# kartikmadhira1/YA_VO

Hardware: AMD Instinct MI355X
Metric: frames/sec (detect+describe+match+PnP) on 1241×376 KITTI stereo; RMSE vs CPU ref (higher is better)
Workload: dtype u8

## Files before the change

### ya_vo_amd/csrc/yavo_kernels.hip

```cpp
#include <hip/hip_runtime.h>
#include <stdint.h>
#include <stdlib.h>
#include <string.h>

#include "yavo_xlane.h"
#include "yavo_internal.h"


namespace yavo {

__device__ __forceinline__ int lane_id() { return (int)(threadIdx.x & 63); }

__device__ __forceinline__ int wave_incl_scan(int v) {
    v += __builtin_amdgcn_update_dpp(0, v, 0x111, 0xf, 0xf, false);
    v += __builtin_amdgcn_update_dpp(0, v, 0x112, 0xf, 0xf, false);
    v += __builtin_amdgcn_update_dpp(0, v, 0x114, 0xf, 0xf, false);
    v += __builtin_amdgcn_update_dpp(0, v, 0x118, 0xf, 0xf, false);
    v += __builtin_amdgcn_update_dpp(0, v, 0x142, 0xa, 0xf, false);
    v += __builtin_amdgcn_update_dpp(0, v, 0x143, 0xc, 0xf, false);
    return v;
}

template <int NT>
__device__ __forceinline__ int block_excl_scan(int v, int* s_tmp, int* total) {
    const int lane = lane_id();
    const int wave = (int)threadIdx.x >> 6;
    constexpr int NW = NT / 64;
    int incl = wave_incl_scan(v);
    if (lane == 63) s_tmp[wave] = incl;
    __syncthreads();
    if (wave == 0) {
        int w = lane < NW ? s_tmp[lane] : 0;
        int wi = wave_incl_scan(w);
        if (lane < NW) s_tmp[lane] = wi - w;
        if (lane == NW - 1) s_tmp[NW] = wi;
    }
    __syncthreads();
    int res = s_tmp[wave] + incl - v;
    if (total) *total = s_tmp[NW];
    __syncthreads();
    return res;
}

#define YV_RING_DR {0, 1, 2, 3, 3, 3, 2, 1, 0, -1, -2, -3, -3, -3, -2, -1}
#define YV_RING_DC {-3, -3, -2, -1, 0, 1, 2, 3, 3, 3, 2, 1, 0, -1, -2, -3}

__device__ __forceinline__ float cv_hypotf(float a, float b) {
    a = fabsf(a);
    b = fabsf(b);
    if (a > b) {
        b /= a;
        return a * sqrtf(1.0f + b * b);
    }
    if (b > 0.0f) {
        a /= b;
        return b * sqrtf(1.0f + a * a);
    }
    return 0.0f;
}

__device__ __forceinline__ float eig_hypotf(float x, float y) {
    x = fabsf(x);
    y = fabsf(y);
    if (isinf(x) || isinf(y)) return __builtin_inff();
    if (isnan(x) || isnan(y)) return __builtin_nanf("");
    const float p = x > y ? x : y;
    if (p == 0.0f) return 0.0f;
    const float qp = (y < x ? y : x) / p;
    return p * sqrtf(1.0f + qp * qp);
}

__device__ void eig_selfadjoint2(float m00, float m01, float m11, float& w0, float& w1) {
    float scale = fabsf(m00);
    if (fabsf(m01) > scale) scale = fabsf(m01);
    if (fabsf(m11) > scale) scale = fabsf(m11);
    if (scale == 0.0f) scale = 1.0f;
    float d0 = m00 / scale, d1 = m11 / scale, e = m01 / scale;
    int iter = 0, ok = 1;
    while (true) {
        if (fabsf(e) < 1.17549435082228750797e-38f) {
            e = 0.0f;
        } else {
            const float se = 8388608.0f * e;
            if (se * se <= (fabsf(d0) + fabsf(d1))) e = 0.0f;
        }
        if (e == 0.0f) break;
        if (++iter > 60) { ok = 0; break; }
        const float td = (d0 - d1) * 0.5f;
        float mu = d1;
        if (td == 0.0f) {
            mu -= fabsf(e);
        } else {
            const float e2 = e * e;
            const float h = eig_hypotf(td, e);
            if (e2 == 0.0f) mu -= e / ((td + (td > 0.0f ? h : -h)) / e);
            else mu -= e2 / (td + (td > 0.0f ? h : -h));
        }
        const float x = d0 - mu, z = e;
        float c, sn;
        if (x == 0.0f) {
            c = 0.0f;
            sn = z < 0.0f ? 1.0f : -1.0f;
        } else if (fabsf(x) > fabsf(z)) {
            const float t = z / x;
            float u = sqrtf(1.0f + t * t);
            if (x < 0.0f) u = -u;
            c = 1.0f / u;
            sn = -t * c;
        } else {
            const float t = x / z;
            float u = sqrtf(1.0f + t * t);
            if (z < 0.0f) u = -u;
            sn = -1.0f / u;
            c = -t * sn;
        }
        const float sdk = sn * d0 + c * e;
        const float dkp1 = sn * e + c * d1;
        const float nd0 = c * (c * d0 - sn * e) - sn * (c * e - sn * d1);
        const float nd1 = sn * sdk + c * dkp1;
        const float ne = c * sdk - sn * dkp1;
        d0 = nd0;
        d1 = nd1;
        e = ne;
    }
    if (ok && d1 < d0) { const float t = d0; d0 = d1; d1 = t; }
    d0 *= scale;
    d1 *= scale;
    w0 = d1;
    w1 = d0;
}

__device__ __forceinline__ float harris_response(float a, float b, float d, int eig) {
    float w0 = a, w1 = d;
    if (eig == 1) {
        eig_selfadjoint2(a, b, d, w0, w1);
    } else if (!(fabsf(b) <= 1.1920928955078125e-07f)) {
        const float p = b;
        const float y = (float)((double)(w1 - w0) * 0.5);
        float t = fabsf(y) + cv_hypotf(p, y);
        float s = cv_hypotf(p, t);
        s = p / s;
        t = (p / t) * p;
        if (y < 0.0f) { s = -s; t = -t; }
        w0 -= t;
        w1 += t;
    }
    if (eig != 1 && w0 < w1) { float tmp = w0; w0 = w1; w1 = tmp; }
    const float prod = w0 * w1;
    const float sum = w1 + w0;
    const double sq = (double)sum * (double)sum;
    const double r = (double)prod - 0.04 * sq;
    return (float)r;
}

__device__ __forceinline__ uint64_t make_key(float resp, uint32_t idx) {
    if (resp == 0.0f) resp = 0.0f;
    uint32_t u = __float_as_uint(resp);
    uint32_t ord = (u & 0x80000000u) ? ~u : (u | 0x80000000u);
    return ((uint64_t)(~ord) << 32) | (uint64_t)idx;
}
__device__ __forceinline__ float key_resp(uint64_t key) {
    uint32_t ord = ~(uint32_t)(key >> 32);
    uint32_t u = (ord & 0x80000000u) ? (ord & 0x7fffffffu) : ~ord;
    return __uint_as_float(u);
}

struct K9 {
    uint32_t k[9];
    uint32_t kh[4][3];
    uint32_t kve[5];
    uint32_t kvo[5];
    int byte2;
    int mfma;
    int hbias;
};

static K9 make_k9(const uint16_t* k9) {
    K9 kw = {};
    uint32_t sum = 0;
    for (int i = 0; i < 9; ++i) {
        kw.k[i] = k9[i];
        sum += k9[i];
    }
    auto tap = [&](int t) -> uint32_t { return (t >= 0 && t <= 8) ? (uint32_t)k9[t] : 0u; };
    for (int j = 0; j < 4; ++j)
        for (int m = 0; m < 3; ++m)
            for (int i = 0; i < 4; ++i) kw.kh[j][m] |= tap(4 * m + i - j) << (8 * i);
    for (int t = 0; t < 5; ++t) {
        kw.kve[t] = tap(2 * t) | (tap(2 * t + 1) << 16);
        kw.kvo[t] = tap(2 * t - 1) | (tap(2 * t) << 16);
    }
    kw.byte2 = sum <= 256 ? 1 : 0;
    uint32_t mx = 0;
    for (int i = 0; i < 9; ++i) mx = k9[i] > mx ? k9[i] : mx;
    kw.mfma = mx <= 127 ? 1 : 0;
    kw.hbias = (int)(128 * sum);
    return kw;
}

__device__ __forceinline__ int reflect101(int p, int len) {
    if (p < 0) p = -p;
    if (p >= len) p = 2 * len - p - 2;
    return p;
}

#ifdef YAVO_LM_PROFILE
constexpr int kDetProfSlots = 131072;
__device__ unsigned long long g_det_prof[kDetProfSlots][6];
#define DP_DECL unsigned long long dp_acc[6] = {0, 0, 0, 0, 0, 0}; unsigned long long dp_t = __builtin_readcyclecounter();
#define DP_MARK(k) do { const unsigned long long t_ = __builtin_readcyclecounter(); dp_acc[k] += t_ - dp_t; dp_t = t_; } while (0)
#define DP_STORE() do { \
        const unsigned slot_ = blockIdx.x; \
        if (threadIdx.x == 0 && slot_ < kDetProfSlots) for (int q_ = 0; q_ < 6; ++q_) g_det_prof[slot_][q_] = dp_acc[q_]; \
    } while (0)
#else
#define DP_DECL
#define DP_MARK(k) do {} while (0)
#define DP_STORE() do {} while (0)
#endif
#ifdef YAVO_LM_PROFILE
constexpr int kBriefProfSlots = 16384;
__device__ unsigned long long g_brief_prof[kBriefProfSlots][6];
#define BP_DECL unsigned long long bp_acc[4] = {0, 0, 0, 0}; unsigned long long bp_t = __builtin_readcyclecounter(); \
    const unsigned long long bp_rt0 = __builtin_amdgcn_s_memrealtime();
#define BP_MARK(k) do { const unsigned long long t_ = __builtin_readcyclecounter(); bp_acc[k] += t_ - bp_t; bp_t = t_; } while (0)
#define BP_STORE() do { \
        if (threadIdx.x == 0 && blockIdx.x < kBriefProfSlots) { \
            g_brief_prof[blockIdx.x][0] = bp_acc[0] + bp_acc[1]; g_brief_prof[blockIdx.x][1] = bp_acc[2]; \
            g_brief_prof[blockIdx.x][2] = bp_rt0; \
            g_brief_prof[blockIdx.x][3] = __builtin_amdgcn_s_memrealtime(); \
            g_brief_prof[blockIdx.x][4] = (unsigned long long)__builtin_amdgcn_s_getreg(0xF804); \
            g_brief_prof[blockIdx.x][5] = (unsigned long long)__builtin_amdgcn_s_getreg(0xF814); \
        } \
    } while (0)
#else
#define BP_DECL
#define BP_MARK(k) do {} while (0)
#define BP_STORE() do {} while (0)
#endif
constexpr int FT_W = kFastTileW;
constexpr int FT_H = kFastTileH;
constexpr int FT_R = 4;
constexpr int FT_LW = FT_W + 2 * FT_R;
constexpr int FT_LH = FT_H + 2 * FT_R;

template <bool kBlur>
__global__ __launch_bounds__(256) void detect_kernel(const uint8_t* __restrict__ imgs, int H, int W, int stride,
                                                     int64_t pitch, int thr, int eig, uint64_t* __restrict__ cand_keys,
                                                     int64_t cap, uint32_t* __restrict__ cand_count, K9 kw,
                                                     uint8_t* __restrict__ blur) {
    __shared__ __align__(16) uint8_t tile[FT_LH * FT_LW];
    constexpr int kPreDw = FT_W * FT_H / 2, kHbufDw = kBlur ? (FT_LH / 2) * FT_W : 0;
    __shared__ __align__(16) uint32_t s_share[kPreDw > kHbufDw ? kPreDw : kHbufDw];
    uint16_t* s_pre = reinterpret_cast<uint16_t*>(s_share);
    uint32_t* hbuf = s_share;
    __shared__ uint16_t s_pos[FT_W * FT_H];
    __shared__ uint32_t s_n, s_npre, s_base;
    __shared__ uint32_t s_band[4 * 9];
    DP_DECL
    const int ntx = (W + FT_W - 1) / FT_W, nty = (H + FT_H - 1) / FT_H;
    const int lb = xcd_swizzle((int)blockIdx.x, (int)gridDim.x);
    const int img = lb / (ntx * nty), tyx = lb - img * (ntx * nty);
    const int r0 = (tyx / ntx) * FT_H, c0 = (tyx % ntx) * FT_W;
    const uint8_t* src = imgs + (int64_t)img * pitch;
    const int tid = threadIdx.x;
    const int lane = lane_id();
    const int wave = tid >> 6;
    if (tid == 0) {
        s_n = 0;
        s_npre = 0;
    }
    if (kBlur && tid < 4 * 9) {
        const int r = tid / 9, M = tid - 9 * r - 3;
        uint32_t v = 0;
#pragma unroll
        for (int j = 0; j < 4; ++j)
#pragma unroll
            for (int m = 0; m < 3; ++m)
                if (r == j && M == m) v = kw.kh[j][m];
        s_band[tid] = v;
    }

    {
        constexpr int kDw = FT_LW / 4;
        constexpr int kSlots = FT_LH * kDw;
        constexpr int kPer = (kSlots + 255) / 256;
        const bool interior = (c0 >= FT_R) && (c0 + FT_W + FT_R <= W) && (r0 >= FT_R) && (r0 + FT_H + FT_R < H);
        uint32_t v[kPer];
        if (interior) {
            const uint8_t* base = src + (int64_t)(r0 - FT_R) * stride + (c0 - FT_R);
            const int lr0 = tid / kDw, j0 = tid - lr0 * kDw;
            uint32_t off = (uint32_t)(lr0 * stride + 4 * j0);
            int j = j0;
            const uint32_t step = (uint32_t)(14 * stride + 16), wrap = (uint32_t)(15 * stride - 56);
            const uint32_t last = (uint32_t)((kSlots - 1) / kDw * stride + 4 * ((kSlots - 1) % kDw));
#pragma unroll
            for (int u = 0; u < kPer; ++u) {
                const uint32_t o = (256 * u + 255 >= kSlots && tid + 256 * u >= kSlots) ? last : off;
                __builtin_memcpy(&v[u], base + o, 4);
                const bool c = j + 4 >= kDw;
                off += c ? wrap : step;
                j += c ? 4 - kDw : 4;
            }
        } else {
#pragma unroll
            for (int u = 0; u < kPer; ++u) {
                const int t = min(tid + 256 * u, kSlots - 1);
                const int lr = t / kDw, j = t - lr * kDw;
                const int r = reflect101(min(max(r0 - FT_R + lr, -(H - 1)), 2 * H - 2), H);
                const uint8_t* row = src + (int64_t)r * stride;
                const int cc = c0 - FT_R + 4 * j;
                if (cc >= 0 && cc + 4 <= W) {
                    __builtin_memcpy(&v[u], row + cc, 4);
                } else {
                    uint32_t w = 0;
#pragma unroll
                    for (int b = 0; b < 4; ++b)
                        w |= (uint32_t)row[reflect101(min(max(cc + b, -(W - 1)), 2 * W - 2), W)] << (8 * b);
                    v[u] = w;
                }
            }
        }
        uint32_t* tile32 = reinterpret_cast<uint32_t*>(tile);
#pragma unroll
        for (int u = 0; u < kPer; ++u) {
            const int t = tid + 256 * u;
            if (t < kSlots) tile32[t] = v[u];
        }
    }
    __syncthreads();
    DP_MARK(0);

    constexpr int ring_dr[16] = YV_RING_DR;
    constexpr int ring_dc[16] = YV_RING_DC;
    const uint32_t neg_thr = (uint32_t)(-thr);
    const int tx = lane;
    const int ty = __builtin_amdgcn_readfirstlane(wave);
    const int c = c0 + tx;
    constexpr int kRowIters = FT_H / 4;
    uint32_t row_ok = 0;
#pragma unroll
    for (int u = 0; u < kRowIters; ++u) row_ok |= (uint32_t)((unsigned)(r0 + ty + 4 * u - 4) < (unsigned)(H - 8)) << u;
    uint32_t nmask = 0;
    const uint8_t* wbase = &tile[(ty + FT_R - 3) * FT_LW + tx + FT_R - 3];
#pragma unroll
    for (int u = kRowIters - 1; u >= 0; --u) {
        const uint8_t* t0 = wbase + 4 * u * FT_LW;
        const uint32_t cent = t0[3 * FT_LW + 3];
        auto d = [&](int k) {
            return __builtin_amdgcn_sad_u8(cent, (uint32_t)t0[(ring_dr[k] + 3) * FT_LW + ring_dc[k] + 3], neg_thr);
        };
        const uint32_t v = (d(0) | d(4)) | (d(8) | d(11));
        nmask = __builtin_amdgcn_alignbit(nmask, v, 31);
    }
    uint32_t pmask = (unsigned)(c - 4) < (unsigned)(W - 8) ? (~nmask & row_ok) : 0u;
    {
        const int cnt = __popc(pmask);
        const int incl = wave_incl_scan(cnt);
        const int total = __shfl(incl, 63, 64);
        uint32_t base = 0;
        if (lane == 0 && total > 0) base = atomicAdd(&s_npre, (uint32_t)total);
        base = __shfl(base, 0, 64);
        uint32_t off = base + (uint32_t)(incl - cnt);
        while (pmask) {
            const int u = __builtin_ctz(pmask);
            s_pre[off++] = (uint16_t)((ty + 4 * u) * FT_W + tx);
            pmask &= pmask - 1;
        }
    }
    __syncthreads();
    DP_MARK(1);
    const uint32_t npre = s_npre;
    for (uint32_t i0 = 0; i0 < npre; i0 += 256) {
        const uint32_t i = i0 + tid;
        bool cand = false;
        int pos = 0;
        if (i < npre) {
            pos = s_pre[i];
            const uint8_t* t0 = &tile[((pos >> 6) + FT_R - 3) * FT_LW + (pos & 63) + FT_R - 3];
            const uint32_t cent = t0[3 * FT_LW + 3];
            uint32_t sim = 0;
#pragma unroll
            for (int k = 0; k < 16; ++k)
                sim = __builtin_amdgcn_alignbit(
                    sim, __builtin_amdgcn_sad_u8(cent, (uint32_t)t0[(ring_dr[k] + 3) * FT_LW + ring_dc[k] + 3], neg_thr),
                    31);
            const uint32_t mask = ~sim & 0xFFFFu;
            const uint32_t a2 = mask & (mask >> 1);
            const uint32_t a4 = a2 & (a2 >> 2);
            const uint32_t a8 = a4 & (a4 >> 4);
            const uint32_t a12 = a8 & (a4 >> 8);
            cand = a12 != 0u;
        }
        const uint64_t bal = __ballot(cand);
        if (bal == 0) continue;
        const int leader = __ffsll((long long)bal) - 1;
        uint32_t base = 0;
        if (lane == leader) base = atomicAdd(&s_n, (uint32_t)__popcll(bal));
        base = __shfl(base, leader, 64);
        if (cand) s_pos[base + (uint32_t)__popcll(bal & ((1ull << lane) - 1ull))] = (uint16_t)pos;
    }
    __syncthreads();
    DP_MARK(2);
    const uint32_t n = s_n;
    if (tid == 0 && n > 0) s_base = atomicAdd(&cand_count[img], n);
    if (kBlur && kw.mfma) {
        typedef int dt_v4i __attribute__((ext_vector_type(4)));
        const int n = lane & 15, g = lane >> 4;
        dt_v4i B;
#pragma unroll
        for (int jj = 0; jj < 4; ++jj) {
            const int M = 4 * g + jj - (n >> 2);
            B[jj] = (M >= -3 && M <= 5) ? (int)s_band[(n & 3) * 9 + M + 3] : 0;
        }
        const dt_v4i C = {kw.hbias, kw.hbias, kw.hbias, kw.hbias};
        const int rb = ty;
        const uint8_t* arow = &tile[(16 * rb + n) * FT_LW + 16 * g];
#pragma unroll
        for (int cb = 0; cb < 4; ++cb) {
            const uint2 lo = *reinterpret_cast<const uint2*>(arow + 16 * cb);
            const uint2 hi = *reinterpret_cast<const uint2*>(arow + 16 * cb + 8);
            const dt_v4i A = {(int)(lo.x ^ 0x80808080u), (int)(lo.y ^ 0x80808080u), (int)(hi.x ^ 0x80808080u),
                              (int)(hi.y ^ 0x80808080u)};
            const dt_v4i acc = __builtin_amdgcn_mfma_i32_16x16x64_i8(A, B, C, 0, 0, 0);
            const int q = 8 * rb + 2 * g, x = 16 * cb + n;
            hbuf[q * FT_W + x] = (uint32_t)acc[0] | ((uint32_t)acc[1] << 16);
            hbuf[(q + 1) * FT_W + x] = (uint32_t)acc[2] | ((uint32_t)acc[3] << 16);
        }
    } else if (kBlur) {
        const uint32_t* trow = reinterpret_cast<const uint32_t*>(tile);
        constexpr int kItems = (FT_LH / 2) * (FT_W / 4);
        for (int i = tid; i < kItems; i += 256) {
            const int q = i >> 4, xq = (i & 15) * 4;
            uint32_t hv[2][4];
#pragma unroll
            for (int h = 0; h < 2; ++h) {
                const uint32_t* wr = trow + ((2 * q + h) * FT_LW >> 2) + (xq >> 2);
                const uint32_t d0 = wr[0], d1 = wr[1], d2 = wr[2];
#pragma unroll
                for (int j = 0; j < 4; ++j) {
                    uint32_t acc = __builtin_amdgcn_udot4(d0, kw.kh[j][0], 0u, false);
                    acc = __builtin_amdgcn_udot4(d1, kw.kh[j][1], acc, false);
                    hv[h][j] = __builtin_amdgcn_udot4(d2, kw.kh[j][2], acc, false);
                }
            }
            *reinterpret_cast<uint4*>(&hbuf[q * FT_W + xq]) =
                make_uint4(hv[0][0] | (hv[1][0] << 16), hv[0][1] | (hv[1][1] << 16), hv[0][2] | (hv[1][2] << 16),
                           hv[0][3] | (hv[1][3] << 16));
        }
    }
    __syncthreads();
    DP_MARK(3);
    if (n > 0) {
        uint64_t* out = cand_keys + (int64_t)img * cap + s_base;
        for (uint32_t i = tid; i < n; i += 256) {
            const int pos = s_pos[i];
            const int prr = pos >> 6, ptx = pos & 63;
            const uint8_t* t0 = &tile[(prr + FT_R - 2) * FT_LW + ptx + FT_R - 2];
            int sxx = 0, sxy = 0, syy = 0;
#pragma unroll
            for (int ii = -1; ii <= 1; ++ii) {
#pragma unroll
                for (int j = -1; j <= 1; ++j) {
                    const uint8_t* q = t0 + (ii + 2) * FT_LW + j + 2;
                    const int pmm = q[-FT_LW - 1], pm0 = q[-FT_LW], pmp = q[-FT_LW + 1];
                    const int p0m = q[-1], p0p = q[1];
                    const int ppm = q[FT_LW - 1], pp0 = q[FT_LW], ppp = q[FT_LW + 1];
                    const int gx = (pmp - pmm) + 2 * (p0p - p0m) + (ppp - ppm);
                    const int gy = (ppm - pmm) + 2 * (pp0 - pm0) + (ppp - pmp);
                    sxx += gx * gx;
                    sxy += gx * gy;
                    syy += gy * gy;
                }
            }
            const float resp = harris_response((float)sxx, (float)sxy, (float)syy, eig);
            out[i] = make_key(resp, (uint32_t)((r0 + prr) * W + (c0 + ptx)));
        }
    }
    DP_MARK(4);
    if (kBlur) {
        typedef unsigned short us2 __attribute__((ext_vector_type(2)));
        const int bp = blur_pitch(W);
        uint8_t* dst = blur + (int64_t)img * H * bp;
        for (int i = tid; i < (FT_H / 2) * (FT_W / 4); i += 256) {
            const int m = i >> 4, xq = (i & 15) * 4;
            uint4 P[5];
#pragma unroll
            for (int t = 0; t < 5; ++t) {
                typedef unsigned int u32x4 __attribute__((ext_vector_type(4)));
                typedef const volatile __attribute__((address_space(3))) u32x4 lds_u32x4;
                const u32x4 q = *(lds_u32x4*)(&s_share[(m + t) * FT_W + xq]);
                P[t] = make_uint4(q.x, q.y, q.z, q.w);
            }
            uint32_t ev[4], od[4];
#pragma unroll
            for (int j = 0; j < 4; ++j) {
                auto col = [&](const uint4& q) { return j == 0 ? q.x : j == 1 ? q.y : j == 2 ? q.z : q.w; };
                uint32_t e = 1u << 15, o = 1u << 15;
#pragma unroll
                for (int t = 0; t < 5; ++t) {
                    e = __builtin_amdgcn_udot2(__builtin_bit_cast(us2, col(P[t])), __builtin_bit_cast(us2, kw.kve[t]), e, false);
                    o = __builtin_amdgcn_udot2(__builtin_bit_cast(us2, col(P[t])), __builtin_bit_cast(us2, kw.kvo[t]), o, false);
                }
                ev[j] = e;
                od[j] = o;
            }
            uint32_t w0, w1;
            if (kw.byte2) {
                w0 = __builtin_amdgcn_perm(__builtin_amdgcn_perm(ev[3], ev[2], 0x0c0c0602u),
                                           __builtin_amdgcn_perm(ev[1], ev[0], 0x0c0c0602u), 0x05040100u);
                w1 = __builtin_amdgcn_perm(__builtin_amdgcn_perm(od[3], od[2], 0x0c0c0602u),
                                           __builtin_amdgcn_perm(od[1], od[0], 0x0c0c0602u), 0x05040100u);
            } else {
                w0 = w1 = 0;
#pragma unroll
                for (int j = 0; j < 4; ++j) {
                    w0 |= min(ev[j] >> 16, 255u) << (8 * j);
                    w1 |= min(od[j] >> 16, 255u) << (8 * j);
                }
            }
            const int r = r0 + 2 * m, c = c0 + xq;
            if (r < H) *reinterpret_cast<uint32_t*>(&dst[(int64_t)r * bp + c]) = w0;
            if (r + 1 < H) *reinterpret_cast<uint32_t*>(&dst[(int64_t)(r + 1) * bp + c]) = w1;
        }
    }
    DP_MARK(5);
    DP_STORE();
}

void launch_fast_harris(const uint8_t* imgs, int n_images, int H, int W, int stride, int64_t pitch,
                        int thr, int eig, uint64_t* cand_keys, int64_t cap, uint32_t* cand_count, hipStream_t s) {
    dim3 grid(((W + FT_W - 1) / FT_W) * ((H + FT_H - 1) / FT_H) * n_images);
    K9 kw = {};
    hipLaunchKernelGGL(detect_kernel<false>, grid, dim3(256), 0, s, imgs, H, W, stride, pitch, thr, eig, cand_keys,
                       cap, cand_count, kw, (uint8_t*)nullptr);
}

void launch_detect_blur(const uint8_t* imgs, int n_images, int H, int W, int stride, int64_t pitch, int thr,
                        int eig, uint64_t* cand_keys, int64_t cap, uint32_t* cand_count, const uint16_t* k9_host,
                        uint8_t* blur, hipStream_t s) {
    dim3 grid(((W + FT_W - 1) / FT_W) * ((H + FT_H - 1) / FT_H) * n_images);
    const K9 kw = make_k9(k9_host);
    hipLaunchKernelGGL(detect_kernel<true>, grid, dim3(256), 0, s, imgs, H, W, stride, pitch, thr, eig, cand_keys, cap,
                       cand_count, kw, blur);
}

constexpr int BL_W = 64, BL_H = 32, BL_R = 4;
constexpr int BL_LW = BL_W + 2 * BL_R;
constexpr int BL_LH = BL_H + 2 * BL_R;

__global__ __launch_bounds__(256) void blur9_kernel(const uint8_t* __restrict__ imgs, int H, int W, int stride,
                                                    int64_t pitch, K9 kw, uint8_t* __restrict__ blur) {
    __shared__ uint8_t tin[BL_LH * BL_LW];
    __shared__ uint32_t th[BL_LH * BL_W];
    const int img = blockIdx.z;
    const int r0 = blockIdx.y * BL_H, c0 = blockIdx.x * BL_W;
    const uint8_t* src = imgs + (int64_t)img * pitch;
    const int tid = threadIdx.x;
    for (int i = tid; i < BL_LH * BL_LW; i += 256) {
        const int lr = i / BL_LW, lc = i - lr * BL_LW;
        const int r = reflect101(min(max(r0 - BL_R + lr, -(H - 1)), 2 * H - 2), H);
        const int c = reflect101(min(max(c0 - BL_R + lc, -(W - 1)), 2 * W - 2), W);
        tin[i] = src[(int64_t)r * stride + c];
    }
    __syncthreads();
    for (int i = tid; i < BL_LH * BL_W; i += 256) {
        const int lr = i >> 6, lc = i & 63;
        const uint8_t* q = &tin[lr * BL_LW + lc];
        uint32_t acc = 0;
#pragma unroll
        for (int j = 0; j < 9; ++j) acc += kw.k[j] * (uint32_t)q[j];
        th[i] = acc;
    }
    __syncthreads();
    const int tx = tid & 63, ty = tid >> 6;
    const int c = c0 + tx;
    for (int rr = ty; rr < BL_H; rr += 4) {
        const int r = r0 + rr;
        uint32_t acc = 0;
#pragma unroll
        for (int i = 0; i < 9; ++i) acc += kw.k[i] * th[(rr + i) * BL_W + tx];
        uint32_t v = (acc + (1u << 15)) >> 16;
        if (r < H && c < W) blur[(int64_t)img * blur_image_bytes(H, W) + (int64_t)r * blur_pitch(W) + c] = (uint8_t)(v > 255u ? 255u : v);
    }
}

void launch_blur9(const uint8_t* imgs, int n_images, int H, int W, int stride, int64_t pitch,
                  const uint16_t* k9_host, uint8_t* blur, hipStream_t s) {
    const K9 kw = make_k9(k9_host);
    dim3 grid((W + BL_W - 1) / BL_W, (H + BL_H - 1) / BL_H, n_images);
    hipLaunchKernelGGL(blur9_kernel, grid, dim3(256), 0, s, imgs, H, W, stride, pitch, kw, blur);
}

constexpr int TK_NT = 1024;

__device__ __forceinline__ bool brief_boundary(int row, int col, int H, int W) {
    return !(col - 8 < 0 || col + 8 > W) && !(row - 8 < 0 || row + 8 > H);
}

__host__ __device__ constexpr int bank_classes(int nb) { return nb <= kBandCounters / 32 ? 32 : 1; }

template <int NT, class RcAt>
__device__ void boundary_compact(RcAt rc_at, int K, int H, int W, int32_t* kp_src, int32_t* kp_count,
                                 int32_t* kp_band, int32_t* band_off, int* s_tmp, int* s_band) {
    const int tid = threadIdx.x;
    const int nb = (H + kBandRows - 1) / kBandRows;
    const int C = bank_classes(nb), nbc = nb * C;
    const int LS = brief_lds_stride(W);
    auto bucket = [&](int row, int col) -> int {
        const int band = row / kBandRows;
        const int cls = C == 1 ? 0 : ((((row - band * kBandRows + 8) * LS + col) >> 2) & 31);
        return band * C + cls;
    };
    for (int b = tid; b < nbc; b += NT) s_band[b] = 0;
    __syncthreads();
    int base = 0;
    for (int pass = 0; pass < 2; ++pass) {
        base = 0;
        for (int c0 = 0; c0 < K; c0 += 4 * NT) {
            int flags[4];
            int2 rcs[4];
            int cnt = 0;
#pragma unroll
            for (int u = 0; u < 4; ++u) {
                const int i = c0 + tid * 4 + u;
                flags[u] = 0;
                rcs[u] = make_int2(0, 0);
                if (i < K) {
                    rcs[u] = rc_at(i);
                    flags[u] = brief_boundary(rcs[u].x, rcs[u].y, H, W) ? 1 : 0;
                }
                cnt += flags[u];
            }
            int total = 0;
            int off = base + block_excl_scan<NT>(cnt, s_tmp, &total);
#pragma unroll
            for (int u = 0; u < 4; ++u) {
                const int i = c0 + tid * 4 + u;
                if (flags[u]) {
                    const int bk = bucket(rcs[u].x, rcs[u].y);
                    if (pass == 0) {
                        reinterpret_cast<int4*>(kp_src)[off] = make_int4(rcs[u].x, rcs[u].y, i, 0);
                        atomicAdd(&s_band[bk], 1);
                    } else {
                        const int pos = atomicAdd(&s_band[bk], 1);
                        reinterpret_cast<int4*>(kp_band)[pos] = make_int4(rcs[u].x, rcs[u].y, i, off);
                    }
                    off++;
                }
            }
            base += total;
        }
        __syncthreads();
        if (pass == 0) {
            int acc = 0;
            for (int b0 = 0; b0 < nbc; b0 += NT) {
                const int j = b0 + tid;
                const int c = j < nbc ? s_band[j] : 0;
                int tot = 0;
                const int first = acc + block_excl_scan<NT>(c, s_tmp, &tot);
                if (j < nbc) {
                    s_band[j] = first;
                    if (j % C == 0) band_off[j / C] = first;
                }
                acc += tot;
            }
            if (tid == 0) band_off[nb] = acc;
        }
        __syncthreads();
    }
    if (tid == 0) *kp_count = base;
}

constexpr int TK_SEL_NT = 512;
static_assert(TK_SEL_NT >= 256 && TK_SEL_NT % 64 == 0, "the radix-select histogram scan uses the first 256 threads");
template <int NT>
__global__ __launch_bounds__(NT) void topk_kernel(const uint64_t* __restrict__ cand_keys, int64_t cap,
                                                     uint32_t* __restrict__ cand_count, uint32_t* __restrict__ cand_seen,
                                                     int H, int W, int max_kp, int keep, int32_t* __restrict__ det_rc,
                                                     float* __restrict__ det_resp, int32_t* __restrict__ det_count,
                                                     int32_t* __restrict__ kp_src, int32_t* __restrict__ kp_count,
                                                     int32_t* __restrict__ kp_band, int32_t* __restrict__ band_off) {
    __shared__ uint64_t s_keys[kMaxKp];
    __shared__ uint32_t s_hist[256];
    __shared__ int s_tmp[40];
    __shared__ int s_band[kBandCounters];
    __shared__ uint64_t s_prefix, s_mask;
    __shared__ int s_krem, s_done, s_n;

    const int img = blockIdx.x;
    const int tid = threadIdx.x;
    const uint64_t* keys = cand_keys + (int64_t)img * cap;
    int64_t C64 = (int64_t)cand_count[img];
    if (C64 > cap) C64 = cap;
    const int C = (int)C64;
    const int K = C < keep ? C : keep;
    __syncthreads();
    if (tid == 0) {
        cand_seen[img] = (uint32_t)C;
        cand_count[img] = 0;
    }
    int32_t* rc_out = det_rc + (int64_t)img * max_kp * 2;
    float* resp_out = det_resp + (int64_t)img * max_kp;

    if (K == 0) {
        const int nb = (H + kBandRows - 1) / kBandRows;
        for (int b = tid; b <= nb; b += NT) band_off[(int64_t)img * (kMaxBands + 1) + b] = 0;
        if (tid == 0) { det_count[img] = 0; kp_count[img] = 0; }
        return;
    }
    uint64_t sel_mask = 0, sel_prefix = ~0ull;
    if (C > K) {
        if (tid == 0) { s_prefix = 0; s_mask = 0; s_krem = K; s_done = 0; }
        __syncthreads();
        for (int shift = 56; shift >= 0; shift -= 8) {
            const uint64_t pm = s_mask, pp = s_prefix;
            const int krem = s_krem;
            if (tid < 256) s_hist[tid] = 0;
            __syncthreads();
            for (int i = tid; i < C; i += NT) {
                const uint64_t k = keys[i];
                if ((k & pm) == pp) atomicAdd(&s_hist[(k >> shift) & 255u], 1u);
            }
            __syncthreads();
            int h = 0, incl = 0;
            if (tid < 256) {
                h = (int)s_hist[tid];
                incl = wave_incl_scan(h);
                if ((tid & 63) == 63) s_tmp[tid >> 6] = incl;
            }
            __syncthreads();
            if (tid < 256) {
                int base = 0;
                for (int w = 0; w < (tid >> 6); ++w) base += s_tmp[w];
                incl += base;
                if (incl >= krem && incl - h < krem) {
                    const int nk = krem - (incl - h);
                    s_prefix = pp | ((uint64_t)tid << shift);
                    s_mask = pm | (0xFFull << shift);
                    s_krem = nk;
                    s_done = (h == nk);
                }
            }
            __syncthreads();
            if (s_done) break;
        }
        sel_mask = s_mask;
        sel_prefix = s_prefix;
    }
    if (tid == 0) s_n = 0;
    __syncthreads();
    for (int i = tid; i < C; i += NT) {
        const uint64_t k = keys[i];
        if ((k & sel_mask) <= sel_prefix) {
            const int p = atomicAdd(&s_n, 1);
            if (p < kMaxKp) s_keys[p] = k;
        }
    }
    __syncthreads();
    int P2 = 1;
    while (P2 < K) P2 <<= 1;
    for (int i = K + tid; i < P2; i += NT) s_keys[i] = ~0ull;
    __syncthreads();
    for (int size = 2; size <= P2; size <<= 1) {
        for (int stride = size >> 1; stride > 0; stride >>= 1) {
            for (int t = tid; t < (P2 >> 1); t += NT) {
                const int i = 2 * t - (t & (stride - 1));
                const int j = i + stride;
                const bool up = ((i & size) == 0);
                const uint64_t a = s_keys[i], b = s_keys[j];
                if ((a > b) == up) { s_keys[i] = b; s_keys[j] = a; }
            }
            __syncthreads();
        }
    }
    for (int i = tid; i < K; i += NT) {
        const uint64_t k = s_keys[i];
        const uint32_t idx = (uint32_t)k;
        const int row = (int)(idx / (uint32_t)W), col = (int)(idx - (uint32_t)row * (uint32_t)W);
        rc_out[2 * i] = row;
        rc_out[2 * i + 1] = col;
// ... 758 lines not shown
```

Baseline: 245,700.

## Compute separable Gaussian blur entirely with MFMA in detect kernel

When the blur kernel is normalized (sum 256) with small taps, the horizontal pass is done by MFMA into registers and the vertical pass is also done by MFMA, with the intermediate split into low and high byte planes so it fits the int8 path. The result is staged in swizzled shared memory and written straight to the blur output, and the kernel returns early, skipping the separate vertical-blur pass and one LDS round trip of the horizontal buffer. Harris scoring is moved into a lambda so both paths can share it. The MFMA path is now restricted to kernels whose taps sum to 256; other kernels fall back to the udot4 path. The byte-split arithmetic adds risk of rounding mismatches against the CPU reference.

```diff
diff --git a/ya_vo_amd/csrc/yavo_kernels.hip b/ya_vo_amd/csrc/yavo_kernels.hip
--- a/ya_vo_amd/csrc/yavo_kernels.hip
+++ b/ya_vo_amd/csrc/yavo_kernels.hip
@@ -193,7 +193,7 @@
     kw.byte2 = sum <= 256 ? 1 : 0;
     uint32_t mx = 0;
     for (int i = 0; i < 9; ++i) mx = k9[i] > mx ? k9[i] : mx;
-    kw.mfma = mx <= 127 ? 1 : 0;
+    kw.mfma = (mx <= 127 && sum == 256) ? 1 : 0;
     kw.hbias = (int)(128 * sum);
     return kw;
 }
@@ -256,7 +256,8 @@
     uint32_t* hbuf = s_share;
     __shared__ uint16_t s_pos[FT_W * FT_H];
     __shared__ uint32_t s_n, s_npre, s_base;
-    __shared__ uint32_t s_band[4 * 9];
+    constexpr int kBandM = 19;
+    __shared__ uint32_t s_band[4 * kBandM];
     DP_DECL
     const int ntx = (W + FT_W - 1) / FT_W, nty = (H + FT_H - 1) / FT_H;
     const int lb = xcd_swizzle((int)blockIdx.x, (int)gridDim.x);
@@ -270,8 +271,8 @@
         s_n = 0;
         s_npre = 0;
     }
-    if (kBlur && tid < 4 * 9) {
-        const int r = tid / 9, M = tid - 9 * r - 3;
+    if (kBlur && tid < 4 * kBandM) {
+        const int r = tid / kBandM, M = tid - kBandM * r - 3;
         uint32_t v = 0;
 #pragma unroll
         for (int j = 0; j < 4; ++j)
@@ -403,56 +404,8 @@
     __syncthreads();
     DP_MARK(2);
     const uint32_t n = s_n;
-    if (tid == 0 && n > 0) s_base = atomicAdd(&cand_count[img], n);
-    if (kBlur && kw.mfma) {
-        typedef int dt_v4i __attribute__((ext_vector_type(4)));
-        const int n = lane & 15, g = lane >> 4;
-        dt_v4i B;
-#pragma unroll
-        for (int jj = 0; jj < 4; ++jj) {
-            const int M = 4 * g + jj - (n >> 2);
-            B[jj] = (M >= -3 && M <= 5) ? (int)s_band[(n & 3) * 9 + M + 3] : 0;
-        }
-        const dt_v4i C = {kw.hbias, kw.hbias, kw.hbias, kw.hbias};
-        const int rb = ty;
-        const uint8_t* arow = &tile[(16 * rb + n) * FT_LW + 16 * g];
-#pragma unroll
-        for (int cb = 0; cb < 4; ++cb) {
-            const uint2 lo = *reinterpret_cast<const uint2*>(arow + 16 * cb);
-            const uint2 hi = *reinterpret_cast<const uint2*>(arow + 16 * cb + 8);
-            const dt_v4i A = {(int)(lo.x ^ 0x80808080u), (int)(lo.y ^ 0x80808080u), (int)(hi.x ^ 0x80808080u),
-                              (int)(hi.y ^ 0x80808080u)};
-            const dt_v4i acc = __builtin_amdgcn_mfma_i32_16x16x64_i8(A, B, C, 0, 0, 0);
-            const int q = 8 * rb + 2 * g, x = 16 * cb + n;
-            hbuf[q * FT_W + x] = (uint32_t)acc[0] | ((uint32_t)acc[1] << 16);
-            hbuf[(q + 1) * FT_W + x] = (uint32_t)acc[2] | ((uint32_t)acc[3] << 16);
-        }
-    } else if (kBlur) {
-        const uint32_t* trow = reinterpret_cast<const uint32_t*>(tile);
-        constexpr int kItems = (FT_LH / 2) * (FT_W / 4);
-        for (int i = tid; i < kItems; i += 256) {
-            const int q = i >> 4, xq = (i & 15) * 4;
-            uint32_t hv[2][4];
-#pragma unroll
-            for (int h = 0; h < 2; ++h) {
-                const uint32_t* wr = trow + ((2 * q + h) * FT_LW >> 2) + (xq >> 2);
-                const uint32_t d0 = wr[0], d1 = wr[1], d2 = wr[2];
-#pragma unroll
-                for (int j = 0; j < 4; ++j) {
-                    uint32_t acc = __builtin_amdgcn_udot4(d0, kw.kh[j][0], 0u, false);
-                    acc = __builtin_amdgcn_udot4(d1, kw.kh[j][1], acc, false);
-                    hv[h][j] = __builtin_amdgcn_udot4(d2, kw.kh[j][2], acc, false);
-                }
-            }
-            *reinterpret_cast<uint4*>(&hbuf[q * FT_W + xq]) =
-                make_uint4(hv[0][0] | (hv[1][0] << 16), hv[0][1] | (hv[1][1] << 16), hv[0][2] | (hv[1][2] << 16),
-                           hv[0][3] | (hv[1][3] << 16));
-        }
-    }
-    __syncthreads();
-    DP_MARK(3);
-    if (n > 0) {
-        uint64_t* out = cand_keys + (int64_t)img * cap + s_base;
+    auto harris = [&](uint32_t base) {
+        uint64_t* out = cand_keys + (int64_t)img * cap + base;
         for (uint32_t i = tid; i < n; i += 256) {
             const int pos = s_pos[i];
             const int prr = pos >> 6, ptx = pos & 63;
@@ -476,7 +429,86 @@
             const float resp = harris_response((float)sxx, (float)sxy, (float)syy, eig);
             out[i] = make_key(resp, (uint32_t)((r0 + prr) * W + (c0 + ptx)));
         }
-    }
+    };
+    if (kBlur && kw.mfma) {
+        if (tid == 0 && n > 0) s_base = atomicAdd(&cand_count[img], n);
+        typedef int dt_v4i __attribute__((ext_vector_type(4)));
+        const int nn = lane & 15, g = lane >> 4;
+        const uint32_t* band = &s_band[(nn & 3) * kBandM + 3 - (nn >> 2)];
+        const dt_v4i B = {(int)band[4 * g], (int)band[4 * g + 1], (int)band[4 * g + 2], (int)band[4 * g + 3]};
+        const dt_v4i Z = {0, 0, 0, 0};
+        const int cb = ty;
+        const uint8_t* arow = &tile[nn * FT_LW + 16 * cb + 16 * g];
+        dt_v4i Hlo, Hhi;
+#pragma unroll
+        for (int rb = 0; rb < 4; ++rb) {
+            const uint2 lo = *reinterpret_cast<const uint2*>(arow + 16 * rb * FT_LW);
+            const uint2 hi = *reinterpret_cast<const uint2*>(arow + 16 * rb * FT_LW + 8);
+            const dt_v4i A = {(int)(lo.x ^ 0x80808080u), (int)(lo.y ^ 0x80808080u), (int)(hi.x ^ 0x80808080u),
+                              (int)(hi.y ^ 0x80808080u)};
+            const dt_v4i acc = __builtin_amdgcn_mfma_i32_16x16x64_i8(A, B, Z, 0, 0, 0);
+            const uint32_t p01 = __builtin_amdgcn_perm((uint32_t)acc[1], (uint32_t)acc[0], 0x05010400u);
+            const uint32_t p23 = __builtin_amdgcn_perm((uint32_t)acc[3], (uint32_t)acc[2], 0x05010400u);
+            Hlo[rb] = (int)(__builtin_amdgcn_perm(p23, p01, 0x05040100u) ^ 0x80808080u);
+            Hhi[rb] = (int)__builtin_amdgcn_perm(p23, p01, 0x07060302u);
+        }
+        const int T0 = (int)band[g], T1 = (int)band[g + 4];
+        const int cv = 257 * kw.hbias + (1 << 15);
+        const dt_v4i Cv = {cv, cv, cv, cv};
+        uint32_t* ostage = &s_share[nn * 16 + ((4 * cb) ^ (nn & 12)) + g];
+#pragma unroll
+        for (int ob = 0; ob < 4; ++ob) {
+            dt_v4i T = {0, 0, 0, 0};
+            T[ob] = T0;
+            if (ob < 3) T[ob + 1] = T1;
+            const dt_v4i vl = __builtin_amdgcn_mfma_i32_16x16x64_i8(Hlo, T, Cv, 0, 0, 0);
+            const dt_v4i vh = __builtin_amdgcn_mfma_i32_16x16x64_i8(Hhi, T, Z, 0, 0, 0);
+            uint32_t v[4];
+#pragma unroll
+            for (int i = 0; i < 4; ++i) v[i] = ((uint32_t)vh[i] << 8) + (uint32_t)vl[i];
+            ostage[ob * 16 * 16] = __builtin_amdgcn_perm(__builtin_amdgcn_perm(v[3], v[2], 0x0c0c0602u),
+                                                         __builtin_amdgcn_perm(v[1], v[0], 0x0c0c0602u), 0x05040100u);
+        }
+        __syncthreads();
+        if (tid < FT_H * 4) {
+            const int R = tid >> 2, q = tid & 3;
+            const int bp = blur_pitch(W);
+            if (r0 + R < H)
+                *reinterpret_cast<uint4*>(blur + ((int64_t)img * H + r0 + R) * bp + c0 + 16 * (q ^ ((R >> 2) & 3))) =
+                    *reinterpret_cast<const uint4*>(&s_share[R * 16 + 4 * q]);
+        }
+        DP_MARK(3);
+        if (n > 0) harris(s_base);
+        DP_MARK(4);
+        DP_STORE();
+        return;
+    }
+    if (tid == 0 && n > 0) s_base = atomicAdd(&cand_count[img], n);
+    if (kBlur) {
+        const uint32_t* trow = reinterpret_cast<const uint32_t*>(tile);
+        constexpr int kItems = (FT_LH / 2) * (FT_W / 4);
+        for (int i = tid; i < kItems; i += 256) {
+            const int q = i >> 4, xq = (i & 15) * 4;
+            uint32_t hv[2][4];
+#pragma unroll
+            for (int h = 0; h < 2; ++h) {
+                const uint32_t* wr = trow + ((2 * q + h) * FT_LW >> 2) + (xq >> 2);
+                const uint32_t d0 = wr[0], d1 = wr[1], d2 = wr[2];
+#pragma unroll
+                for (int j = 0; j < 4; ++j) {
+                    uint32_t acc = __builtin_amdgcn_udot4(d0, kw.kh[j][0], 0u, false);
+                    acc = __builtin_amdgcn_udot4(d1, kw.kh[j][1], acc, false);
+                    hv[h][j] = __builtin_amdgcn_udot4(d2, kw.kh[j][2], acc, false);
+                }
+            }
+            *reinterpret_cast<uint4*>(&hbuf[q * FT_W + xq]) =
+                make_uint4(hv[0][0] | (hv[1][0] << 16), hv[0][1] | (hv[1][1] << 16), hv[0][2] | (hv[1][2] << 16),
+                           hv[0][3] | (hv[1][3] << 16));
+        }
+    }
+    __syncthreads();
+    DP_MARK(3);
+    if (n > 0) harris(s_base);
     DP_MARK(4);
     if (kBlur) {
         typedef unsigned short us2 __attribute__((ext_vector_type(2)));
```

After: 250,900 (median of 6 runs). 1.02x the previous value.
